# anerisheth19/CNN-MobileNet-V1-implementation-on-AWS-FPGA-using-OpenCL

Measured on AMD Instinct MI355X. Metric: images/sec MobileNet-V1 1.0x224 fp32, batch 256; per-stage HBM GB/s vs roofline, higher is better.
Workload: dtype f32

## Files before the change

cnn-mobilenet-v1-implementation-on-aws-fpga-using-opencl_amd/csrc/mbn_f32_stem.hip:

```cpp
#include "mbn_internal.h"
#include "mbn_epilogue.h"
#include "mbn_x6.h"

namespace {

constexpr int TH = MBN_STEM_TH, TW = MBN_STEM_TW;
constexpr int CR = TH + 2, CC = TW + 2;
constexpr int PR = 2 * CR + 1;
constexpr int PROW = 112;
constexpr int PROWPAD = 4;

struct StemArgs {

    float *out;
    const float *in, *w1, *s1, *b1, *wd, *s2, *b2, *wp, *s3, *b3;
    const uint8_t *in8;
    int batch, rows, cols;
    int oh, ow;
    int tiles_y, tiles_x;
    unsigned ntiles;
};

template <int C1>
__device__ __forceinline__ int swz(int row, int chunk)
{
    if (C1 == 32) return (row << 5) + (((chunk ^ (row >> 1)) & 7) << 2);
    return (row << 4) + (((chunk ^ (row >> 2)) & 3) << 2);
}
template <int C1>
__device__ __forceinline__ int swzb(int row, int slot)
{
    if (C1 == 32) return (row << 4) + (((slot ^ (row >> 2)) & 3) << 2);
    return (row << 3) + (((slot ^ (row >> 3)) & 1) << 2);
}
__device__ __forceinline__ f4 fma4(float x, f4 w, f4 acc) { return __builtin_elementwise_fma(f4{ x, x, x, x }, w, acc); }
__device__ __forceinline__ f4 fma4v(f4 x, f4 w, f4 acc) { return __builtin_elementwise_fma(x, w, acc); }

constexpr int PAIRS = PROW / 2;
constexpr int NPF = (PR * PAIRS + 255) / 256;

__device__ __forceinline__ void patch_load(const StemArgs &a, unsigned t, int tid, f2 (&pf)[NPF])
{
    const int tx = (int)(t % (unsigned)a.tiles_x);
    const unsigned q0 = t / (unsigned)a.tiles_x;
    const int ty = (int)(q0 % (unsigned)a.tiles_y);
    const long n = q0 / (unsigned)a.tiles_y;
    const long img = n * a.rows * a.cols * 3;
    const int iy0 = 2 * (TH * ty - 1), fx0 = 6 * (TW * tx - 1), rowf = a.cols * 3;
    const unsigned img_elems = (unsigned)(a.rows * a.cols * 3);
    if (a.in8) {
        const __amdgpu_buffer_rsrc_t rsrc = mbn_make_rsrc(a.in8 + img, img_elems);
#pragma unroll
        for (int k = 0; k < NPF; k++) {
            const int i = tid + k * 256, r = i / PAIRS, j = i % PAIRS;
            const int iy = iy0 + r, fx = fx0 + 2 * j;
            const bool ok = i < PR * PAIRS && iy >= 0 && iy < a.rows && fx >= 0 && fx < rowf;
            const unsigned u = (unsigned short)__builtin_amdgcn_raw_buffer_load_b16(rsrc, ok ? (unsigned)(iy * rowf + fx) : MBN_OOB, 0, 0);
            pf[k] = ok ? f2{ fmaf((float)(u & 0xff), 1.0f / 127.5f, -1.0f), fmaf((float)(u >> 8), 1.0f / 127.5f, -1.0f) } : f2{ 0.f, 0.f };
        }
    } else {
        const __amdgpu_buffer_rsrc_t rsrc = mbn_make_rsrc(a.in + img, img_elems * 4u);
#pragma unroll
        for (int k = 0; k < NPF; k++) {
            const int i = tid + k * 256, r = i / PAIRS, j = i % PAIRS;
            const int iy = iy0 + r, fx = fx0 + 2 * j;
            const bool ok = i < PR * PAIRS && iy >= 0 && iy < a.rows && fx >= 0 && fx < rowf;
            pf[k] = __builtin_bit_cast(f2, __builtin_amdgcn_raw_buffer_load_b64(rsrc, ok ? (unsigned)(iy * rowf + fx) * 4u : MBN_OOB, 0, 0));
        }
    }
}
__device__ __forceinline__ void patch_store(float *in_s, int tid, const f2 (&pf)[NPF])
{
#pragma unroll
    for (int k = 0; k < NPF; k++) {
        const int i = tid + k * 256;
        if (i < PR * PAIRS) *reinterpret_cast<f2 *>(in_s + 2 * i) = pf[k];
    }
}

__device__ __forceinline__ float rbf(float v) { return (float)(__bf16)v; }
__device__ __forceinline__ f4 rbf4(f4 v) { return f4{ rbf(v.x), rbf(v.y), rbf(v.z), rbf(v.w) }; }
template <int C1, int C3, bool BF, int WPE, bool MC = false, int X6 = 0, bool PADC = true>
__global__ __launch_bounds__(256, WPE) void stem_fused_f32(StemArgs a)
{
    static_assert(!MC || BF || C1 == 32, "conv1 on the MFMA: bf16 mode (16x16x32 bf16, split operands), or fp32 alpha = 1 (16x16x4 fp32)");
    constexpr bool MCF = MC && !BF;
    static_assert(X6 == 0 || (!BF && (X6 == 6 || X6 == 9)), "split products: fp32 mode, 6 or 9 of them");
    constexpr int APL = TH * TW * C1 / 2, BPL = C3 * C1 / 2;
    constexpr int MH = C1 / 16;
    constexpr bool WDL = WPE >= 3;
    constexpr int Q1 = C1 / 4;
    constexpr int PB = 3 * Q1 / 4;
    static_assert(CC % PB == 0 && CR * (CC / PB) * Q1 <= 256, "conv1 lane mapping");
    constexpr int NXV = (3 * (2 * PB + 1) + 3) / 4;
    constexpr int PC = 128 * Q1 / 256;
    constexpr int NI = C3 / 32;
    constexpr int KG = C1 / 8;
    constexpr bool BREG = !BF && X6 == 0 && WPE >= 3 && C1 == 32;
    __shared__ __attribute__((aligned(16))) float in_s[PR * PROW + PROWPAD];
    __shared__ __attribute__((aligned(16))) float w1_s[27 * C1];
    constexpr int C1P = (MCF && C1 == 32 && PADC) ? 40 : C1;
    __shared__ __attribute__((aligned(16))) float c1_s[CR * CC * C1P];
    __shared__ __attribute__((aligned(16))) float a_s[X6 ? 3 * APL : TH * TW * C1 / (BF ? 2 : 1)];
    __shared__ __attribute__((aligned(16))) float b_s[BREG ? 4 : X6 ? 3 * BPL : C3 * C1 / (BF ? 2 : 1)];
    __shared__ __attribute__((aligned(16))) float sb_s[4 * C1];
    __shared__ __attribute__((aligned(16))) float wd_s[WDL ? 9 * C1 : 4];

    const int tid = threadIdx.x, lane = tid & 63, wave = tid >> 6, li = lane & 31, lh = lane >> 5;
    const int c4 = tid % Q1;

    for (int i = tid * 4; i < 27 * C1; i += 1024) *reinterpret_cast<f4 *>(w1_s + i) = *reinterpret_cast<const f4 *>(a.w1 + i);
    if (BF) {
        constexpr int SL = C1 / 8;
        if (tid < C3 * SL) {
            const int row = tid / SL, slot = tid % SL, ch = NI == 2 ? 2 * (row & 31) + (row >> 5) : row;
            *reinterpret_cast<f4 *>(b_s + swzb<C1>(row, slot)) =
                *reinterpret_cast<const f4 *>(reinterpret_cast<const __bf16 *>(a.wp) + ch * C1 + slot * 8);
        }
    } else if constexpr (X6 != 0) {
        constexpr int SL = C1 / 8;
        if (tid < C3 * SL) {
            const int row = tid / SL, slot = tid % SL;
            const float *src = a.wp + row * C1 + slot * 8;
            u4 hw, mw, lw;
            mbn_x6_split8(*reinterpret_cast<const f4 *>(src), *reinterpret_cast<const f4 *>(src + 4), hw, mw, lw);
            *reinterpret_cast<u4 *>(b_s + swzb<C1>(row, slot)) = hw;
            *reinterpret_cast<u4 *>(b_s + BPL + swzb<C1>(row, slot)) = mw;
            *reinterpret_cast<u4 *>(b_s + 2 * BPL + swzb<C1>(row, slot)) = lw;
        }
    } else if constexpr (!BREG)
    for (int i = tid; i < C3 * Q1; i += 256) {
        const int row = i / Q1, ch = i % Q1;
        *reinterpret_cast<f4 *>(b_s + swz<C1>(row, ch)) = *reinterpret_cast<const f4 *>(a.wp + row * C1 + ch * 4);
    }
    [[maybe_unused]] f4 bfr[BREG ? KG : 1][NI];
    if constexpr (BREG) {
#pragma unroll
        for (int g = 0; g < KG; g++)
#pragma unroll
            for (int ni = 0; ni < NI; ni++) bfr[g][ni] = *reinterpret_cast<const f4 *>(a.wp + (ni * 32 + (tid & 31)) * C1 + (2 * g + ((tid & 63) >> 5)) * 4);
    }
    if (tid < 4 * C1) {
        const float *src = tid < C1 ? a.s1 : tid < 2 * C1 ? a.b1 : tid < 3 * C1 ? a.s2 : a.b2;
        sb_s[tid] = src[tid & (C1 - 1)];
    }
    f4 wd[WDL ? 1 : 9];
    if constexpr (WDL) {
        for (int i = tid * 4; i < 9 * C1; i += 1024) *reinterpret_cast<f4 *>(wd_s + i) = *reinterpret_cast<const f4 *>(a.wd + i);
    } else {
#pragma unroll
        for (int k = 0; k < 9; k++) wd[k] = *reinterpret_cast<const f4 *>(a.wd + k * C1 + c4 * 4);
    }
    float s3[NI], b3[NI];
#pragma unroll
    for (int ni = 0; ni < NI; ni++) {
        const int ch = (BF && NI == 2) ? 2 * li + ni : ni * 32 + li;
        s3[ni] = a.s3[ch]; b3[ni] = a.b3[ch];
    }

    f2 pf[NPF];
    if (blockIdx.x < a.ntiles) {
        patch_load(a, blockIdx.x, tid, pf);
        patch_store(in_s, tid, pf);
    }
    __syncthreads();

    [[maybe_unused]] int mc_dl[8];
    [[maybe_unused]] unsigned mc_kok = 0;
    [[maybe_unused]] bf8 mc_wh[MH], mc_wl[MH];
    [[maybe_unused]] f4 mc_s1[MH], mc_b1[MH];
    [[maybe_unused]] int mcf_dl[7];
    [[maybe_unused]] float mcf_w[2][7];
    [[maybe_unused]] f4 mcf_s1[2], mcf_b1[2];
    if constexpr (MCF) {
        const int kg = lane >> 4, pc = lane & 15;
#pragma unroll
        for (int t = 0; t < 7; t++) {
            const int k = 4 * t + kg;
            mcf_dl[t] = k < 27 ? (k / 9) * PROW + (k % 9) : 0;
#pragma unroll
            for (int h = 0; h < 2; h++) mcf_w[h][t] = k < 27 ? w1_s[k * C1 + 16 * h + pc] : 0.f;
        }
#pragma unroll
        for (int h = 0; h < 2; h++) {
            mcf_s1[h] = *reinterpret_cast<const f4 *>(sb_s + 16 * h + 4 * kg);
            mcf_b1[h] = *reinterpret_cast<const f4 *>(sb_s + C1 + 16 * h + 4 * kg);
        }
    }
    if constexpr (MC && BF) {
        const int kg = lane >> 4, pc = lane & 15;
        unsigned whb[MH][8], wlb[MH][8];
#pragma unroll
        for (int j = 0; j < 8; j++) {
            const int k = 8 * kg + j;
            mc_dl[j] = (k / 9) * PROW + (k % 9);
            if (k < 27) mc_kok |= 1u << j;
#pragma unroll
            for (int h = 0; h < MH; h++) {
                const float w = k < 27 ? w1_s[k * C1 + 16 * h + pc] : 0.f;
                const unsigned wb = __builtin_bit_cast(unsigned, w) & 0xffff0000u;
                whb[h][j] = wb;
                wlb[h][j] = __builtin_bit_cast(unsigned, w - __builtin_bit_cast(float, wb));
            }
        }
#pragma unroll
        for (int h = 0; h < MH; h++) {
            u4 ph, pl;
#pragma unroll
            for (int i = 0; i < 4; i++) {
                ph[i] = (whb[h][2 * i] >> 16) | (whb[h][2 * i + 1] & 0xffff0000u);
                pl[i] = (wlb[h][2 * i] >> 16) | (wlb[h][2 * i + 1] & 0xffff0000u);
            }
            mc_wh[h] = __builtin_bit_cast(bf8, ph);
            mc_wl[h] = __builtin_bit_cast(bf8, pl);
            mc_s1[h] = *reinterpret_cast<const f4 *>(sb_s + 16 * h + 4 * kg);
            mc_b1[h] = *reinterpret_cast<const f4 *>(sb_s + C1 + 16 * h + 4 * kg);
        }
    }

    const int bpg = tid / Q1, br = bpg / (CC / PB), bc = (bpg % (CC / PB)) * PB;
    const int cy = (tid / Q1) / (TW / PC), cx = ((tid / Q1) % (TW / PC)) * PC;

    for (unsigned t = blockIdx.x; t < a.ntiles; t += gridDim.x) {
        const int tx = (int)(t % (unsigned)a.tiles_x);
        const unsigned q0 = t / (unsigned)a.tiles_x;
        const int ty = (int)(q0 % (unsigned)a.tiles_y);
        const long n = q0 / (unsigned)a.tiles_y;
        const unsigned tnext = t + gridDim.x;
        if (tnext < a.ntiles) patch_load(a, tnext, tid, pf);

        __builtin_amdgcn_s_setprio(2);
        if constexpr (MCF) {
            const int kg = lane >> 4, pc = lane & 15;
#pragma unroll 1
            for (int bi = 0; bi < 3; bi++) {
                const int blk = wave * 3 + bi;
                const int q = 16 * blk + pc, p = min(q, CR * CC - 1);
                const int r = (p * 3641) >> 16, c = p - r * CC;
                const float *src = in_s + (2 * r) * PROW + 6 * c;
                float xv[7];
#pragma unroll
                for (int t = 0; t < 7; t++) xv[t] = src[mcf_dl[t]];
                if (kg == 3) xv[6] = 0.f;
                const int oy = TH * ty - 1 + r, ox = TW * tx - 1 + c;
                const bool inside = oy >= 0 && oy < a.oh && ox >= 0 && ox < a.ow;
#pragma unroll
                for (int h = 0; h < 2; h++) {
                    f4 acc = f4{ 0.f, 0.f, 0.f, 0.f };
#pragma unroll
                    for (int t = 0; t < 7; t++) acc = __builtin_amdgcn_mfma_f32_16x16x4f32(mcf_w[h][t], xv[t], acc, 0, 0, 0);
                    const f4 v = inside ? mbn_bn_relu6(acc, mcf_s1[h], mcf_b1[h]) : f4{ 0.f, 0.f, 0.f, 0.f };
                    if (q < CR * CC) *reinterpret_cast<f4 *>(c1_s + q * C1P + 16 * h + 4 * kg) = v;
                }
            }
        } else
        if constexpr (MC) {
            const int kg = lane >> 4, pc = lane & 15;
#pragma unroll 1
            for (int bi = 0; bi < 3; bi++) {
                const int blk = wave * 3 + bi;
                const int q = 16 * blk + pc, p = min(q, CR * CC - 1);
                const int r = (p * 3641) >> 16, c = p - r * CC;
                const float *src = in_s + (2 * r) * PROW + 6 * c;
                unsigned xb[8], lb[8];
#pragma unroll
                for (int j = 0; j < 8; j++) {
                    const float x = ((mc_kok >> j) & 1u) ? src[mc_dl[j]] : 0.f;
                    xb[j] = __builtin_bit_cast(unsigned, x) & 0xffff0000u;
                    lb[j] = __builtin_bit_cast(unsigned, x - __builtin_bit_cast(float, xb[j]));
                }
                u4 ph, pl;
#pragma unroll
                for (int i = 0; i < 4; i++) {
                    ph[i] = (xb[2 * i] >> 16) | (xb[2 * i + 1] & 0xffff0000u);
                    pl[i] = (lb[2 * i] >> 16) | (lb[2 * i + 1] & 0xffff0000u);
                }
                const bf8 xh = __builtin_bit_cast(bf8, ph), xl = __builtin_bit_cast(bf8, pl);
                const int oy = TH * ty - 1 + r, ox = TW * tx - 1 + c;
                const bool inside = oy >= 0 && oy < a.oh && ox >= 0 && ox < a.ow;
#pragma unroll
                for (int h = 0; h < MH; h++) {
                    f4 acc = f4{ 0.f, 0.f, 0.f, 0.f };
                    acc = __builtin_amdgcn_mfma_f32_16x16x32_bf16(mc_wl[h], xh, acc, 0, 0, 0);
                    acc = __builtin_amdgcn_mfma_f32_16x16x32_bf16(mc_wh[h], xl, acc, 0, 0, 0);
                    acc = __builtin_amdgcn_mfma_f32_16x16x32_bf16(mc_wh[h], xh, acc, 0, 0, 0);
                    const f4 v = inside ? rbf4(mbn_bn_relu6(acc, mc_s1[h], mc_b1[h])) : f4{ 0.f, 0.f, 0.f, 0.f };
                    if (q < CR * CC) *reinterpret_cast<f4 *>(c1_s + q * C1 + 16 * h + 4 * kg) = v;
                }
            }
        } else
        if (bpg < CR * (CC / PB)) {
            f4 acc[PB];
#pragma unroll
            for (int p = 0; p < PB; p++) acc[p] = f4{ 0.f, 0.f, 0.f, 0.f };
#pragma unroll 1
            for (int ky = 0; ky < 3; ky++) {
                const float *row = in_s + (2 * br + ky) * PROW + (2 * bc) * 3;
                float x[4 * NXV];
                if constexpr (PB == 6) {
#pragma unroll
                    for (int j = 0; j < NXV; j++) {
                        const f4 t = *reinterpret_cast<const f4 *>(row + 4 * j);
                        x[4 * j] = t.x; x[4 * j + 1] = t.y; x[4 * j + 2] = t.z; x[4 * j + 3] = t.w;
                    }
                } else {
#pragma unroll
                    for (int j = 0; j < 2 * NXV - 1; j++) {
                        const f2 t = *reinterpret_cast<const f2 *>(row + 2 * j);
                        x[2 * j] = t.x; x[2 * j + 1] = t.y;
                    }
                }
#pragma unroll
                for (int kx = 0; kx < 3; kx++)
#pragma unroll
                    for (int ci = 0; ci < 3; ci++) {
                        const f4 w = *reinterpret_cast<const f4 *>(w1_s + ((ky * 3 + kx) * 3 + ci) * C1 + c4 * 4);
#pragma unroll
                        for (int p = 0; p < PB; p++) acc[p] = fma4(x[(2 * p + kx) * 3 + ci], w, acc[p]);
                    }
            }
            const int oy = TH * ty - 1 + br, ox = TW * tx - 1 + bc;
            const bool rowok = oy >= 0 && oy < a.oh;
            const f4 s1 = *reinterpret_cast<const f4 *>(sb_s + c4 * 4), b1 = *reinterpret_cast<const f4 *>(sb_s + C1 + c4 * 4);
#pragma unroll
            for (int p = 0; p < PB; p++) {
                f4 v = (rowok && ox + p >= 0 && ox + p < a.ow) ? mbn_bn_relu6(acc[p], s1, b1) : f4{ 0.f, 0.f, 0.f, 0.f };
                if (BF) v = rbf4(v);
                *reinterpret_cast<f4 *>(c1_s + (br * CC + bc + p) * C1 + c4 * 4) = v;
            }
        }
        __syncthreads();
        if (tnext < a.ntiles) patch_store(in_s, tid, pf);

        {
            f4 acc[PC];
#pragma unroll
            for (int p = 0; p < PC; p++) acc[p] = f4{ 0.f, 0.f, 0.f, 0.f };
#pragma unroll
            for (int dy = 0; dy < 3; dy++) {
                f4 v[PC + 2];
#pragma unroll
                for (int j = 0; j < PC + 2; j++) v[j] = *reinterpret_cast<const f4 *>(c1_s + ((cy + dy) * CC + cx + j) * C1P + c4 * 4);
#pragma unroll
                for (int dx = 0; dx < 3; dx++) {
                    f4 wt;
                    if constexpr (WDL) wt = *reinterpret_cast<const f4 *>(wd_s + (dy * 3 + dx) * C1 + c4 * 4);
                    else wt = wd[dy * 3 + dx];
#pragma unroll
                    for (int p = 0; p < PC; p++) acc[p] = fma4v(v[p + dx], wt, acc[p]);
                }
            }
            const f4 s2 = *reinterpret_cast<const f4 *>(sb_s + 2 * C1 + c4 * 4), b2 = *reinterpret_cast<const f4 *>(sb_s + 3 * C1 + c4 * 4);
#pragma unroll
            for (int p = 0; p < PC; p++) {
                const f4 v = mbn_bn_relu6(acc[p], s2, b2);
                if (BF) {
                    const int row = cy * TW + cx + p;
                    *reinterpret_cast<bf4 *>(a_s + swzb<C1>(row, c4 >> 1) + 2 * (c4 & 1)) = bf4{ (__bf16)v.x, (__bf16)v.y, (__bf16)v.z, (__bf16)v.w };
                } else if constexpr (X6 != 0) {
                    const int o = swzb<C1>(cy * TW + cx + p, c4 >> 1) + 2 * (c4 & 1);
                    u2 hw, mw, lw;
                    mbn_x6_split4(v, hw, mw, lw);
                    *reinterpret_cast<u2 *>(a_s + o) = hw;
                    *reinterpret_cast<u2 *>(a_s + APL + o) = mw;
                    *reinterpret_cast<u2 *>(a_s + 2 * APL + o) = lw;
                } else *reinterpret_cast<f4 *>(a_s + swz<C1>(cy * TW + cx + p, c4)) = v;
            }
        }
        __syncthreads();

        __builtin_amdgcn_s_setprio(0);
        f16v acc[NI];
#pragma unroll
        for (int ni = 0; ni < NI; ni++)
#pragma unroll
            for (int r = 0; r < 16; r++) acc[ni][r] = 0.f;
        if constexpr (BF) {
#pragma unroll
            for (int ks = 0; ks < C1 / 16; ks++) {
                const f4 av = *reinterpret_cast<const f4 *>(a_s + swzb<C1>(wave * 32 + li, 2 * ks + lh));
#pragma unroll
                for (int ni = 0; ni < NI; ni++) {
                    const f4 bv = *reinterpret_cast<const f4 *>(b_s + swzb<C1>(ni * 32 + li, 2 * ks + lh));
                    acc[ni] = __builtin_amdgcn_mfma_f32_32x32x16_bf16(__builtin_bit_cast(bf8, av), __builtin_bit_cast(bf8, bv), acc[ni], 0, 0, 0);
                }
            }
            const __amdgpu_buffer_rsrc_t orsrc = mbn_make_rsrc(reinterpret_cast<__bf16 *>(a.out) + n * a.oh * a.ow * C3, (unsigned)(a.oh * a.ow * C3 * 2));
            const unsigned lane_off = (unsigned)(4 * lh * C3) * 2u + (unsigned)li * (NI == 2 ? 4u : 2u);
#pragma unroll
            for (int r = 0; r < 16; r++) {
                const int y = TH * ty + 2 * __builtin_amdgcn_readfirstlane(wave) + (r >> 3), x = TW * tx + (r & 3) + 8 * ((r >> 2) & 1);
                const unsigned soff = (unsigned)((y * a.ow + x) * C3) * 2u;
                if constexpr (NI == 2) {
                    const float v0 = mbn_relu6(fmaf(acc[0][r], s3[0], b3[0])), v1 = mbn_relu6(fmaf(acc[1][r], s3[1], b3[1]));
                    __builtin_amdgcn_raw_buffer_store_b32(__builtin_bit_cast(unsigned, bf2{ (__bf16)v0, (__bf16)v1 }), orsrc, lane_off, soff, 0);
                } else {
                    __builtin_amdgcn_raw_buffer_store_b16(__builtin_bit_cast(unsigned short, (__bf16)mbn_relu6(fmaf(acc[0][r], s3[0], b3[0]))), orsrc, lane_off, soff, 0);
                }
            }
        } else {
        if constexpr (X6 != 0) {
            constexpr int pa9[9] = { 2, 2, 1, 2, 0, 1, 1, 0, 0 }, pb9[9] = { 2, 1, 2, 0, 2, 1, 0, 1, 0 };
            constexpr int pa6[6] = { 2, 0, 1, 1, 0, 0 }, pb6[6] = { 0, 2, 1, 0, 1, 0 };
#pragma unroll
            for (int ks = 0; ks < C1 / 16; ks++) {
                f4 av[3], bv[3][NI];
#pragma unroll
                for (int pl = 0; pl < 3; pl++) {
                    av[pl] = *reinterpret_cast<const f4 *>(a_s + pl * APL + swzb<C1>(wave * 32 + li, 2 * ks + lh));
#pragma unroll
                    for (int ni = 0; ni < NI; ni++) bv[pl][ni] = *reinterpret_cast<const f4 *>(b_s + pl * BPL + swzb<C1>(ni * 32 + li, 2 * ks + lh));
                }
#pragma unroll
                for (int q = 0; q < X6; q++)
#pragma unroll
                    for (int ni = 0; ni < NI; ni++)
                        acc[ni] = __builtin_amdgcn_mfma_f32_32x32x16_bf16(__builtin_bit_cast(bf8, av[X6 == 6 ? pa6[q % 6] : pa9[q]]),
                                                                          __builtin_bit_cast(bf8, bv[X6 == 6 ? pb6[q % 6] : pb9[q]][ni]), acc[ni], 0, 0, 0);
            }
        } else
#pragma unroll
        for (int g = 0; g < KG; g++) {
            const int chunk = 2 * g + lh;
            const f4 av = *reinterpret_cast<const f4 *>(a_s + swz<C1>(wave * 32 + li, chunk));
            f4 bv[NI];
#pragma unroll
            for (int ni = 0; ni < NI; ni++) {
                if constexpr (BREG) bv[ni] = bfr[g][ni];
                else bv[ni] = *reinterpret_cast<const f4 *>(b_s + swz<C1>(ni * 32 + li, chunk));
            }
#pragma unroll
            for (int s = 0; s < 4; s++)
#pragma unroll
                for (int ni = 0; ni < NI; ni++) acc[ni] = __builtin_amdgcn_mfma_f32_32x32x2f32(av[s], bv[ni][s], acc[ni], 0, 0, 0);
        }
        if constexpr (C1 == 32 && !BREG) {
            float *obase = a.out + ((n * a.oh + TH * ty) * a.ow + TW * tx) * C3;
#pragma unroll
            for (int ni = 0; ni < NI; ni++)
#pragma unroll
                for (int r = 0; r < 16; r++) {
                    const int q = wave * 32 + (r & 3) + 8 * (r >> 2) + 4 * lh;
                    const int y = q >> 4, x = q & 15;
                    obase[((long)y * a.ow + x) * C3 + ni * 32 + li] = mbn_relu6(fmaf(acc[ni][r], s3[ni], b3[ni]));
                }
        } else {
        const __amdgpu_buffer_rsrc_t orsrc = mbn_make_rsrc(a.out + n * a.oh * a.ow * C3, (unsigned)(a.oh * a.ow * C3 * 4));
        const unsigned lane_off = (unsigned)(4 * lh * C3 + li) * 4u;
#pragma unroll
        for (int ni = 0; ni < NI; ni++)
#pragma unroll
            for (int r = 0; r < 16; r++) {
                const int y = TH * ty + 2 * __builtin_amdgcn_readfirstlane(wave) + (r >> 3), x = TW * tx + (r & 3) + 8 * ((r >> 2) & 1);
                const unsigned soff = (unsigned)((y * a.ow + x) * C3 + ni * 32) * 4u;
                __builtin_amdgcn_raw_buffer_store_b32(__builtin_bit_cast(unsigned, mbn_relu6(fmaf(acc[ni][r], s3[ni], b3[ni]))), orsrc, lane_off, soff, 0);
            }
        }
        }
    }
}

}

int mbn_launch_f32_stem(mbn_context *ctx, hipStream_t stream, float *out, const float *in, const float *w1,
                        const float *s1, const float *b1, const float *wd, const float *s2, const float *b2,
                        const float *wp, const float *s3, const float *b3, int batch, int rows, int cols, int c1, int c3, int in_u8, int bf16)
{
    StemArgs a;
    a.in8 = in_u8 ? (const uint8_t *)in : nullptr;
    a.out = out; a.in = in; a.w1 = w1; a.s1 = s1; a.b1 = b1; a.wd = wd; a.s2 = s2; a.b2 = b2; a.wp = wp; a.s3 = s3; a.b3 = b3;
    a.batch = batch; a.rows = rows; a.cols = cols; a.oh = rows / 2; a.ow = cols / 2;
    a.tiles_y = a.oh / TH; a.tiles_x = a.ow / TW;
    a.ntiles = (unsigned)((long)batch * a.tiles_y * a.tiles_x);
    const int wpe_bf = g_mbn_tune.misc == 2 ? 2 : 3;
    const int per_cu = c1 == 16 ? 4 : (bf16 ? wpe_bf : 2);
    long grid = (long)ctx->num_cus * per_cu;
    if (grid > (long)a.ntiles) grid = (long)a.ntiles;
    const dim3 g((unsigned)grid), b(256);
    if (c1 == 32) {
#ifdef MBN_LAB
        if (bf16 && wpe_bf == 3 && g_mbn_tune.conv_variant == 2) hipLaunchKernelGGL((stem_fused_f32<32, 64, true, 3>), g, b, 0, stream, a);
        else if (bf16 && wpe_bf != 3) hipLaunchKernelGGL((stem_fused_f32<32, 64, true, 2>), g, b, 0, stream, a);
        else
#endif
        if (bf16) hipLaunchKernelGGL((stem_fused_f32<32, 64, true, 3, true>), g, b, 0, stream, a);
        else if (g_mbn_tune.pw_emul == 6) hipLaunchKernelGGL((stem_fused_f32<32, 64, false, 2, true, 6>), g, b, 0, stream, a);
        else if (g_mbn_tune.pw_emul == 9) hipLaunchKernelGGL((stem_fused_f32<32, 64, false, 2, true, 9>), g, b, 0, stream, a);
#ifdef MBN_LAB
        else if (g_mbn_tune.conv_variant == 3 || g_mbn_tune.conv_variant == 4) {
            long g3 = (long)ctx->num_cus * (g_mbn_tune.conv_variant == 3 ? 3 : 2);
            if (g3 > (long)a.ntiles) g3 = (long)a.ntiles;
            hipLaunchKernelGGL((stem_fused_f32<32, 64, false, 3>), dim3((unsigned)g3), b, 0, stream, a);
        }
#endif
#ifdef MBN_LAB
        else if (g_mbn_tune.conv_variant == 6) hipLaunchKernelGGL((stem_fused_f32<32, 64, false, 2, true, 0, false>), g, b, 0, stream, a);
        else if (g_mbn_tune.conv_variant == 5) hipLaunchKernelGGL((stem_fused_f32<32, 64, false, 2>), g, b, 0, stream, a);
#endif
        else hipLaunchKernelGGL((stem_fused_f32<32, 64, false, 2, true>), g, b, 0, stream, a);
    } else {
#ifdef MBN_LAB
        if (bf16 && g_mbn_tune.conv_variant == 2) hipLaunchKernelGGL((stem_fused_f32<16, 32, true, 4>), g, b, 0, stream, a);
        else
#endif
        if (bf16) {
            long g5 = (long)ctx->num_cus * 5;
            if (g5 > (long)a.ntiles) g5 = (long)a.ntiles;
            hipLaunchKernelGGL((stem_fused_f32<16, 32, true, 5, true>), dim3((unsigned)g5), b, 0, stream, a);
        }
        else if (g_mbn_tune.pw_emul == 6) hipLaunchKernelGGL((stem_fused_f32<16, 32, false, 4, false, 6>), g, b, 0, stream, a);
        else if (g_mbn_tune.pw_emul == 9) hipLaunchKernelGGL((stem_fused_f32<16, 32, false, 4, false, 9>), g, b, 0, stream, a);
        else hipLaunchKernelGGL((stem_fused_f32<16, 32, false, 4>), g, b, 0, stream, a);
    }
    return MBN_OK;
}
```

Before: 91390.

## Shrink fp32 stem LDS footprint to run three workgroups per CU on large batches

Adds a fp32 MFMA stem variant at three workgroups per CU. It frees LDS by placing the conv1 filter in the A-tile buffer (which needs an extra barrier) and by reducing the c1 channel padding from 40 to 36. The default fp32 path now picks this occupancy-3 form when there are enough tiles per CU, and otherwise falls back to the previous two-per-CU launch. Lab-only variants with channel-paired 8-byte output stores are also added. The trade-off is tighter register and LDS budgets and possibly more bank conflicts from the smaller padding.

```diff
diff --git a/cnn-mobilenet-v1-implementation-on-aws-fpga-using-opencl_amd/csrc/mbn_f32_stem.hip b/cnn-mobilenet-v1-implementation-on-aws-fpga-using-opencl_amd/csrc/mbn_f32_stem.hip
--- a/cnn-mobilenet-v1-implementation-on-aws-fpga-using-opencl_amd/csrc/mbn_f32_stem.hip
+++ b/cnn-mobilenet-v1-implementation-on-aws-fpga-using-opencl_amd/csrc/mbn_f32_stem.hip
@@ -80,9 +80,10 @@
 
 __device__ __forceinline__ float rbf(float v) { return (float)(__bf16)v; }
 __device__ __forceinline__ f4 rbf4(f4 v) { return f4{ rbf(v.x), rbf(v.y), rbf(v.z), rbf(v.w) }; }
-template <int C1, int C3, bool BF, int WPE, bool MC = false, int X6 = 0, bool PADC = true>
+template <int C1, int C3, bool BF, int WPE, bool MC = false, int X6 = 0, bool PADC = true, int EPI = 0>
 __global__ __launch_bounds__(256, WPE) void stem_fused_f32(StemArgs a)
 {
+    static_assert(EPI == 0 || (!BF && X6 == 0 && C1 == 32 && C3 == 64 && EPI <= 2), "channel-paired 8-byte stores: fp32 alpha = 1");
     static_assert(!MC || BF || C1 == 32, "conv1 on the MFMA: bf16 mode (16x16x32 bf16, split operands), or fp32 alpha = 1 (16x16x4 fp32)");
     constexpr bool MCF = MC && !BF;
     static_assert(X6 == 0 || (!BF && (X6 == 6 || X6 == 9)), "split products: fp32 mode, 6 or 9 of them");
@@ -97,14 +98,17 @@
     constexpr int NI = C3 / 32;
     constexpr int KG = C1 / 8;
     constexpr bool BREG = !BF && X6 == 0 && WPE >= 3 && C1 == 32;
+    constexpr bool W1A = MCF && WPE >= 3;
     __shared__ __attribute__((aligned(16))) float in_s[PR * PROW + PROWPAD];
-    __shared__ __attribute__((aligned(16))) float w1_s[27 * C1];
-    constexpr int C1P = (MCF && C1 == 32 && PADC) ? 40 : C1;
+    __shared__ __attribute__((aligned(16))) float w1_own[W1A ? 4 : 27 * C1];
+    constexpr int C1P = (MCF && C1 == 32 && PADC) ? (WPE >= 3 ? 36 : 40) : C1;
     __shared__ __attribute__((aligned(16))) float c1_s[CR * CC * C1P];
     __shared__ __attribute__((aligned(16))) float a_s[X6 ? 3 * APL : TH * TW * C1 / (BF ? 2 : 1)];
     __shared__ __attribute__((aligned(16))) float b_s[BREG ? 4 : X6 ? 3 * BPL : C3 * C1 / (BF ? 2 : 1)];
     __shared__ __attribute__((aligned(16))) float sb_s[4 * C1];
     __shared__ __attribute__((aligned(16))) float wd_s[WDL ? 9 * C1 : 4];
+    static_assert(!W1A || sizeof(a_s) >= 27 * C1 * sizeof(float), "the conv1 filter fits the A tile it borrows");
+    float *const w1_s = W1A ? a_s : w1_own;
 
     const int tid = threadIdx.x, lane = tid & 63, wave = tid >> 6, li = lane & 31, lh = lane >> 5;
     const int c4 = tid % Q1;
@@ -131,14 +135,14 @@
     } else if constexpr (!BREG)
     for (int i = tid; i < C3 * Q1; i += 256) {
         const int row = i / Q1, ch = i % Q1;
-        *reinterpret_cast<f4 *>(b_s + swz<C1>(row, ch)) = *reinterpret_cast<const f4 *>(a.wp + row * C1 + ch * 4);
+        *reinterpret_cast<f4 *>(b_s + swz<C1>(row, ch)) = *reinterpret_cast<const f4 *>(a.wp + (EPI ? mbn_pair_channel(row) : row) * C1 + ch * 4);
     }
     [[maybe_unused]] f4 bfr[BREG ? KG : 1][NI];
     if constexpr (BREG) {
 #pragma unroll
         for (int g = 0; g < KG; g++)
 #pragma unroll
-            for (int ni = 0; ni < NI; ni++) bfr[g][ni] = *reinterpret_cast<const f4 *>(a.wp + (ni * 32 + (tid & 31)) * C1 + (2 * g + ((tid & 63) >> 5)) * 4);
+            for (int ni = 0; ni < NI; ni++) bfr[g][ni] = *reinterpret_cast<const f4 *>(a.wp + (EPI ? 2 * (tid & 31) + ni : ni * 32 + (tid & 31)) * C1 + (2 * g + ((tid & 63) >> 5)) * 4);
     }
     if (tid < 4 * C1) {
         const float *src = tid < C1 ? a.s1 : tid < 2 * C1 ? a.b1 : tid < 3 * C1 ? a.s2 : a.b2;
@@ -154,7 +158,7 @@
     float s3[NI], b3[NI];
 #pragma unroll
     for (int ni = 0; ni < NI; ni++) {
-        const int ch = (BF && NI == 2) ? 2 * li + ni : ni * 32 + li;
+        const int ch = ((BF && NI == 2) || EPI) ? 2 * li + ni : ni * 32 + li;
         s3[ni] = a.s3[ch]; b3[ni] = a.b3[ch];
     }
 
@@ -186,6 +190,7 @@
             mcf_s1[h] = *reinterpret_cast<const f4 *>(sb_s + 16 * h + 4 * kg);
             mcf_b1[h] = *reinterpret_cast<const f4 *>(sb_s + C1 + 16 * h + 4 * kg);
         }
+        if constexpr (W1A) __syncthreads();
     }
     if constexpr (MC && BF) {
         const int kg = lane >> 4, pc = lane & 15;
@@ -434,7 +439,30 @@
 #pragma unroll
                 for (int ni = 0; ni < NI; ni++) acc[ni] = __builtin_amdgcn_mfma_f32_32x32x2f32(av[s], bv[ni][s], acc[ni], 0, 0, 0);
         }
-        if constexpr (C1 == 32 && !BREG) {
+        if constexpr (EPI != 0) {
+            const f2 scx = f2{ s3[0], s3[0] }, scy = f2{ s3[1], s3[1] }, shx = f2{ b3[0], b3[0] }, shy = f2{ b3[1], b3[1] };
+            [[maybe_unused]] float *orow0 = a.out + ((n * a.oh + TH * ty + 2 * wave) * a.ow + TW * tx + 4 * lh) * C3 + 2 * li;
+            [[maybe_unused]] float *orow1 = orow0 + (long)a.ow * C3;
+            [[maybe_unused]] const __amdgpu_buffer_rsrc_t orsrc = mbn_make_rsrc(a.out + n * a.oh * a.ow * C3, (unsigned)(a.oh * a.ow * C3 * 4));
+            [[maybe_unused]] const unsigned lane_off = (unsigned)(4 * lh * C3 + 2 * li) * 4u;
+#pragma unroll
+            for (int r = 0; r < 16; r += 2) {
+                const f2 p0 = __builtin_elementwise_fma(f2{ acc[0][r], acc[0][r + 1] }, scx, shx);
+                const f2 p1 = __builtin_elementwise_fma(f2{ acc[1][r], acc[1][r + 1] }, scy, shy);
+#pragma unroll
+                for (int h = 0; h < 2; h++) {
+                    const int rr = r + h;
+                    const f2 v = f2{ mbn_relu6(h ? p0.y : p0.x), mbn_relu6(h ? p1.y : p1.x) };
+                    if constexpr (EPI == 1) {
+                        *reinterpret_cast<f2 *>(((rr >> 3) ? orow1 : orow0) + ((rr & 3) + 8 * ((rr >> 2) & 1)) * C3) = v;
+                    } else {
+                        const int y = TH * ty + 2 * __builtin_amdgcn_readfirstlane(wave) + (rr >> 3), x = TW * tx + (rr & 3) + 8 * ((rr >> 2) & 1);
+                        const unsigned soff = (unsigned)((y * a.ow + x) * C3) * 4u;
+                        __builtin_amdgcn_raw_buffer_store_b64(__builtin_bit_cast(u2, v), orsrc, lane_off, soff, 0);
+                    }
+                }
+            }
+        } else if constexpr (C1 == 32 && !BREG) {
             float *obase = a.out + ((n * a.oh + TH * ty) * a.ow + TW * tx) * C3;
 #pragma unroll
             for (int ni = 0; ni < NI; ni++)
@@ -458,6 +486,15 @@
         }
         }
     }
+}
+
+constexpr int STEM_F32_WIDE_TILES = 12;
+template <int WPE, int EPI>
+void launch_f32_form(const mbn_context *ctx, hipStream_t stream, const StemArgs &a)
+{
+    long grid = (long)ctx->num_cus * WPE;
+    if (grid > (long)a.ntiles) grid = (long)a.ntiles;
+    hipLaunchKernelGGL((stem_fused_f32<32, 64, false, WPE, true, 0, true, EPI>), dim3((unsigned)grid), dim3(256), 0, stream, a);
 }
 
 }
@@ -487,17 +524,17 @@
         else if (g_mbn_tune.pw_emul == 6) hipLaunchKernelGGL((stem_fused_f32<32, 64, false, 2, true, 6>), g, b, 0, stream, a);
         else if (g_mbn_tune.pw_emul == 9) hipLaunchKernelGGL((stem_fused_f32<32, 64, false, 2, true, 9>), g, b, 0, stream, a);
 #ifdef MBN_LAB
-        else if (g_mbn_tune.conv_variant == 3 || g_mbn_tune.conv_variant == 4) {
-            long g3 = (long)ctx->num_cus * (g_mbn_tune.conv_variant == 3 ? 3 : 2);
-            if (g3 > (long)a.ntiles) g3 = (long)a.ntiles;
-            hipLaunchKernelGGL((stem_fused_f32<32, 64, false, 3>), dim3((unsigned)g3), b, 0, stream, a);
-        }
-#endif
-#ifdef MBN_LAB
         else if (g_mbn_tune.conv_variant == 6) hipLaunchKernelGGL((stem_fused_f32<32, 64, false, 2, true, 0, false>), g, b, 0, stream, a);
         else if (g_mbn_tune.conv_variant == 5) hipLaunchKernelGGL((stem_fused_f32<32, 64, false, 2>), g, b, 0, stream, a);
+        else if (g_mbn_tune.conv_variant == 10) launch_f32_form<2, 0>(ctx, stream, a);
+        else if (g_mbn_tune.conv_variant == 11) launch_f32_form<2, 1>(ctx, stream, a);
+        else if (g_mbn_tune.conv_variant == 12) launch_f32_form<2, 2>(ctx, stream, a);
+        else if (g_mbn_tune.conv_variant == 13) launch_f32_form<3, 0>(ctx, stream, a);
+        else if (g_mbn_tune.conv_variant == 14) launch_f32_form<3, 1>(ctx, stream, a);
+        else if (g_mbn_tune.conv_variant == 15) launch_f32_form<3, 2>(ctx, stream, a);
 #endif
-        else hipLaunchKernelGGL((stem_fused_f32<32, 64, false, 2, true>), g, b, 0, stream, a);
+        else if ((long)a.ntiles >= (long)STEM_F32_WIDE_TILES * ctx->num_cus) launch_f32_form<3, 0>(ctx, stream, a);
+        else launch_f32_form<2, 0>(ctx, stream, a);
     } else {
 #ifdef MBN_LAB
         if (bf16 && g_mbn_tune.conv_variant == 2) hipLaunchKernelGGL((stem_fused_f32<16, 32, true, 4>), g, b, 0, stream, a);
```

After: 92160, median of 6. About the same (+0.8%).
